# ruiminshen/yolo2-pytorch

Hardware: NVIDIA H100
Metric: 416x416 images/sec (higher is better)
Workload: dtype f16

## Files before the change

yolo2-pytorch_b200/b200/engine.py:

```python
import os

import torch

from . import ops

STRICT_KEEP = {'layers1.0': 'aw', 'layers1.2': 'aw', 'layers1.4': 'a', 'passthrough': 'aw', 'layers3.0': 'aw'}
PRECISIONS = ('fast', 'strict')


class OperandCache(dict):

    def fetch(self, key, tensors, build, extra=()):
        ver = tuple((t.data_ptr(), t._version) for t in tensors) + tuple(extra)
        hit = self.get(key)
        if hit is None or hit[0] != ver:
            hit = self[key] = (ver, build())
        return hit[1]


def epilogue_tensors(bn, bias=None):
    ts = () if bias is None else (bias,)
    return ts if bn is None else ts + (bn.weight, bn.bias, bn.running_mean, bn.running_var)


# ... 126 lines not shown

class DarknetEngine(object):
    def __init__(self, dnn):
        def unit(m):
            return ConvUnit(m.conv, m.bn if m.has_bn else None, m.has_act)

        self.units1, self.pools1, self._k1 = [], [], []
        mods = list(dnn.layers1)
        for i, m in enumerate(mods):
            if m.is_pool:
                continue
            self.units1.append(unit(m))
            self.pools1.append(i + 1 < len(mods) and mods[i + 1].is_pool)
            self._k1.append('layers1.%d' % i)
        self.units2 = [unit(m) for m in dnn.layers2 if not m.is_pool]
        self._k2 = ['layers2.%d' % i for i, m in enumerate(dnn.layers2) if not m.is_pool]
        self.unit_pt = unit(dnn.passthrough)
        self.units3 = [unit(m) for m in dnn.layers3]
        self.plans = {}
        if not self.pools1[0]:
            raise RuntimeError('Darknet: layers1.0 must be followed by MaxPool2d (fused first-layer kernel)')
        self.precision = 'fast'
        self.set_precision(os.environ.get('YB_PRECISION', 'fast'))

    def unit_keys(self):
        return self._k1 + self._k2 + ['passthrough', 'layers3.0', 'layers3.1']

    def set_precision(self, precision, keep=None):
        if precision not in PRECISIONS:
            raise ValueError('precision must be one of %s' % (PRECISIONS,))
        keep = STRICT_KEEP if keep is None else keep
        units = dict(zip(self.unit_keys(), self.all_units()))
        for key, u in units.items():
            k = keep.get(key, '') if precision == 'strict' else 'aw'
            u.split_a, u.split_w, u.out_lo = 'a' not in k, 'w' not in k, False
        units[self._k1[0]].split_a = units[self._k1[0]].split_w = False
        units[self._k1[1]].split_a = False
        chain1 = self.units1
        for prev, nxt in zip(chain1[:-1], chain1[1:]):
            prev.out_lo = nxt.split_a
        chain1[-1].out_lo = self.unit_pt.split_a or self.units2[0].split_a
        for prev, nxt in zip(self.units2[:-1], self.units2[1:]):
            prev.out_lo = nxt.split_a
        self.units2[-1].out_lo = self.unit_pt.out_lo = self.units3[0].split_a
        self.units3[0].out_lo = self.units3[1].split_a
        chain1[0].out_lo = False
# ... 30 lines not shown
        if u8:
            b, h, w, c = x.shape
        else:
            b, c, h, w = x.shape
        if c != 3 or h % 32 or w % 32:
            raise ValueError('Darknet expects fp32 [B,3,H,W] or uint8 [B,H,W,3] with H, W multiples of 32, got %s' % (tuple(x.shape),))
        x = x.contiguous() if u8 else x.contiguous().float()
        self.refresh()
        p = self.plan(b, h, w, x.device, plan_id)
        if self.precision == 'strict':
            return self._forward_strict(x, u8, p, conv_flags, collect)

        def conv(u, src, dst, **kw):
            return ops.conv_bn_act(src, u.w16, u.scale, u.shift, u.slope, out=dst, flags=conv_flags, ref=ref, workspace=p.workspace, **kw)

        u0 = self.units1[0]
        conv0 = ops.conv0_u8_bn_leaky_pool if u8 else ops.conv0_bn_leaky_pool
        cur = conv0(x, u0.w16, u0.scale, u0.shift, u0.slope, out=p.a0)
        if collect is not None:
            collect['layers1.0(pooled)'] = cur
        x1 = None
        last1 = self.units1[-1]
        for u, (out, pooled), key in zip(self.units1[1:], p.l1, self._k1[1:]):
            fuse_pool = (pooled is not None and u is not last1 and collect is None and not ref and u.cin == 32 and u.ksize == 3
                         and u.cout <= 64 and (conv_flags & (ops.CONV_NO_SMALLK | ops.CONV_C32_IM2COL)) == 0 and conv_flags < 256)
            if fuse_pool:
                ops.conv_bn_act(cur, u.w16, u.scale, u.shift, u.slope, out=pooled, flags=conv_flags | ops.CONV_POOL2X2)
                cur = pooled
                continue
            conv(u, cur, out)
            if collect is not None:
                collect[key] = out
            x1 = out
            cur = ops.maxpool2x2(out, out=pooled) if pooled is not None else out
        conv(self.unit_pt, x1, p.pt)
        if collect is not None:
            collect['passthrough'] = p.pt
        ops.reorg_f16(p.pt, p.cat, 0)
        cur = ops.maxpool2x2(x1, out=p.x1_pool)
        for u, out, key in zip(self.units2[:-1], p.l2, self._k2):
            conv(u, cur, out)
            if collect is not None:
                collect[key] = out
            cur = out
        conv(self.units2[-1], cur, p.cat, y_ch_off=self.unit_pt.cout * 4)
        conv(self.units3[0], p.cat, p.l3)
        conv(self.units3[1], p.l3, p.feature, out_mode=ops.OUT_F32_NCHW)
        if collect is not None:
            collect['cat'] = p.cat
            collect['layers3.0'] = p.l3
# ... 63 lines not shown
```

yolo2-pytorch_b200/b200/ops.py:

```python
import ctypes

import torch

from . import lib as _l

OUT_F16_NHWC, OUT_F32_NCHW = 0, 1
CONV_A_TILED, CONV_WIDE_N = 1, 2
CONV_NO_STREAMK, CONV_FORCE_STREAMK, CONV_NO_SMALLK, CONV_PLAIN_STORE = 8, 1 << 30, 1 << 28, 1 << 29
CONV_POOL2X2, CONV_C32_IM2COL, CONV_C32_SWAP = 16, 32, 64
FILTER_THRESHOLD, FILTER_FIX, FILTER_NONE = 0, 1, 2


launch_count = 0


def _ck(rc, what):
    global launch_count
    _l.check(rc, what)
    launch_count += 1


def conv_force_bn(bn):
    return bn << 8

# ... 108 lines not shown
        fn_name = 'yb_conv_bn_act_fwd_ws'
    fn = getattr(_l.load(), fn_name)
    args = [_p(x), _p(w), _p(scale), _p(shift), float(slope), _p(out), batch, height, width, cin, cout, k, x_ld, y_ld, y_ch_off, out_mode]
    if fn_name != 'yb_conv_ref_fwd':
        args.append(flags)
    if fn_name == 'yb_conv_bn_act_fwd_ws':
        _req(workspace, torch.uint8, 'workspace')
        args += [_p(workspace), workspace.numel()]
    args.append(_s())
    _ck(fn(*args), fn_name)


def conv_workspace(device='cuda'):
    return torch.zeros(int(_l.load().yb_conv_workspace_bytes()), dtype=torch.uint8, device=device)


CONV_KERNELS = ('conv_igemm_kernel', 'conv_wide_kernel', 'conv_c32_kernel')


def conv_choice(batch, height, width, cin, cout, k, out_mode=OUT_F16_NHWC, flags=0, workspace=True):
    out = (ctypes.c_int * 6)()
    _l.check(_l.load().yb_conv_choice(batch, height, width, cin, cout, k, out_mode, flags, int(bool(workspace)), ctypes.byref(out)),
             'yb_conv_choice')
    return dict(kernel=CONV_KERNELS[out[0]], bk=out[1], bn=out[2], rows=out[3], streamk=bool(out[4]), grid=out[5])


def conv_bn_act(x, w, scale, shift, slope, out=None, out_mode=OUT_F16_NHWC, y_ch_off=0, cin=None, flags=0, ref=False, workspace=None):
    _req(x, torch.float16, 'x'); _req(w, torch.float16, 'w'); _req(scale, torch.float32, 'scale'); _req(shift, torch.float32, 'shift')
    b, h, wd, x_ld = x.shape
    cout, k, _, wcin = w.shape
    cin = wcin if cin is None else cin
    if cin != wcin:
        raise ValueError('weight Cin %d != %d' % (wcin, cin))
    if out is None:
        oh, ow = (h // 2, wd // 2) if (flags & CONV_POOL2X2) else (h, wd)
        out = (torch.empty(b, oh, ow, cout, dtype=torch.float16, device=x.device) if out_mode == OUT_F16_NHWC
               else torch.empty(b, cout, h, wd, dtype=torch.float32, device=x.device))
    if out_mode == OUT_F16_NHWC:
        _req(out, torch.float16, 'out')
        y_ld = out.shape[-1]
    else:
        _req(out, torch.float32, 'out')
        y_ld = 0
    _conv_common('yb_conv_ref_fwd' if ref else 'yb_conv_bn_act_fwd', x, w, scale, shift, slope, out, b, h, wd, cin, cout, k, x_ld, y_ld,
                 y_ch_off, out_mode, flags, workspace=None if ref else workspace)
    return out


def conv2d_out_size(size, k, stride, pad):
    return (size + 2 * pad - k) // stride + 1


def conv2d_choice(batch, height, width, cin, cout, kh, kw, stride=1, pad=(0, 0), out_mode=OUT_F16_NHWC, flags=0, workspace=True):
    out = (ctypes.c_int * 6)()
    _l.check(_l.load().yb_conv2d_choice(batch, height, width, cin, cout, kh, kw, stride, pad[0], pad[1], out_mode, flags, int(bool(workspace)),
                                        ctypes.byref(out)), 'yb_conv2d_choice')
    return dict(kernel=CONV_KERNELS[out[0]], bk=out[1], bn=out[2], rows=out[3], streamk=bool(out[4]), grid=out[5])


def conv2d_bn_act(x, w, scale, shift, slope, stride=1, pad=(0, 0), out=None, out_mode=OUT_F16_NHWC, y_ch_off=0, cin=None, flags=0, workspace=None):
    _req(x, torch.float16, 'x'); _req(w, torch.float16, 'w'); _req(scale, torch.float32, 'scale'); _req(shift, torch.float32, 'shift')
    b, h, wd, x_ld = x.shape
    cout, kh, kw, wcin = w.shape
    cin = wcin if cin is None else cin
    if cin != wcin:
        raise ValueError('weight Cin %d != %d' % (wcin, cin))
    oh, ow = conv2d_out_size(h, kh, stride, pad[0]), conv2d_out_size(wd, kw, stride, pad[1])
    if out is None:
        out = (torch.empty(b, oh, ow, cout, dtype=torch.float16, device=x.device) if out_mode == OUT_F16_NHWC
               else torch.empty(b, cout, oh, ow, dtype=torch.float32, device=x.device))
    if out_mode == OUT_F16_NHWC:
        _req(out, torch.float16, 'out')
        y_ld = out.shape[-1]
    else:
        _req(out, torch.float32, 'out')
        y_ld = 0
    ws_ptr, ws_bytes = (None, 0) if workspace is None else (_p(_req(workspace, torch.uint8, 'workspace')), workspace.numel())
    _ck(_l.load().yb_conv2d_bn_act_fwd(_p(x), _p(w), _p(scale), _p(shift), float(slope), _p(out), b, h, wd, cin, cout, kh, kw, stride, pad[0], pad[1],
                                       x_ld, y_ld, y_ch_off, out_mode, flags, ws_ptr, ws_bytes, _s()), 'yb_conv2d_bn_act_fwd')
    return out
# ... 380 lines not shown
```

yolo2-pytorch_b200/csrc/conv_igemm.cu:

```cuda
#include "yb_common.h"
#include "yb_ptx.cuh"
#include <stdlib.h>

namespace yb {

struct ConvParams {
  int m_total;
  int height, width;
  int cin, cout;
  int kh, kw, pad_h, pad_w, stride;
  int in_h, in_w;
  int kb_per_tap;
  int num_kb;
  int m_tiles, n_tiles;
  int a_im2col;
  const float* scale;
  const float* shift;
  float slope;
  void* y;
  long long y_ld;
  int y_ch_off;
  int out_mode;
  int hw;
  int skip;
// ... 545 lines not shown
      acc_phase ^= 1;
    }
    if (p.tma_store && lane == 0) tma_store_wait<0>();
  }
}

template <int BN, int BK, int MT>
__global__ void __launch_bounds__(kThreads, 1)
conv_igemm_kernel(const __grid_constant__ CUtensorMap tmap_a, const __grid_constant__ CUtensorMap tmap_b,
                  const __grid_constant__ CUtensorMap tmap_y, const ConvParams p) {
  conv_igemm_body<BN, BK, MT, false>(tmap_a, tmap_b, tmap_y, p, PreAct{nullptr, nullptr, 0});
}

template <int BN, int BK, int MT>
__global__ void __launch_bounds__(kThreads, 1)
conv_preact_kernel(const __grid_constant__ CUtensorMap tmap_a, const __grid_constant__ CUtensorMap tmap_b,
                   const __grid_constant__ CUtensorMap tmap_y, const ConvParams p, const PreAct pre) {
  conv_igemm_body<BN, BK, MT, true>(tmap_a, tmap_b, tmap_y, p, pre);
}

constexpr int kWideThreads = 384;
constexpr int kWideRows = 256;
constexpr int kWideBN = 128;

template <int BK>
struct WideCfg {
  static constexpr int kSwizzle = BK * 2;
  static constexpr int kABytes = kWideRows * BK * 2;
  static constexpr int kBBytes = kWideBN * BK * 2;
  static constexpr int kStageBytes = kABytes + kBBytes;
  static constexpr int kOutBytes = 128 * 128;
  static constexpr int kTableBytes = kWideBN * 2 * 4;
  static constexpr int kFixedBytes = 2 * kOutBytes + kTableBytes + 1024  + 256 ;
  static constexpr int kStages = ((kSmemLimit - kFixedBytes) / kStageBytes) > 8 ? 8 : ((kSmemLimit - kFixedBytes) / kStageBytes);
  static constexpr int kSmemBytes = kStages * kStageBytes + kFixedBytes;
  static constexpr int kWsFloats = kWideRows * kWideBN;
  static_assert(kStages >= (BK == 64 ? 4 : 8), "shared memory budget: the epilogue's slices and table must not cost a pipeline stage");
};

template <int BK>
__global__ void __launch_bounds__(kWideThreads, 1)
conv_wide_kernel(const __grid_constant__ CUtensorMap tmap_a, const __grid_constant__ CUtensorMap tmap_b,
                 const __grid_constant__ CUtensorMap tmap_y, const ConvParams p) {
  using Cfg = WideCfg<BK>;
  constexpr int kStages = Cfg::kStages;
  extern __shared__ uint8_t smem_raw[];
  const uint32_t smem_base = (smem_u32(smem_raw) + 1023u) & ~1023u;
  const uint32_t smem_a = smem_base;
  const uint32_t smem_b = smem_base + kStages * Cfg::kABytes;
  const uint32_t smem_o = smem_base + kStages * Cfg::kStageBytes;
  const uint32_t table = smem_o + 2 * Cfg::kOutBytes;
  const uint32_t bar_full = table + Cfg::kTableBytes;
  const uint32_t bar_empty = bar_full + 8 * kStages;
  const uint32_t bar_slice_full = bar_empty + 8 * kStages;
  const uint32_t bar_slice_empty = bar_slice_full + 16;
  const int num_tiles = p.m_tiles * p.n_tiles;
  const int unit_id = static_cast<int>(blockIdx.x);
  const int num_units = static_cast<int>(gridDim.x);

  if (threadIdx.x == 0) {
    for (int i = 0; i < kStages; ++i) {
      mbar_init(bar_full + 8 * i, 1);
      mbar_init(bar_empty + 8 * i, 8);
    }
    for (int c = 0; c < 2; ++c) {
      mbar_init(bar_slice_full + 8 * c, 4);
      mbar_init(bar_slice_empty + 8 * c, 1);
    }
    fence_mbar_init();
    fence_proxy_async_smem();
    tma_prefetch_desc(&tmap_a);
    tma_prefetch_desc(&tmap_b);
    tma_prefetch_desc(&tmap_y);
  }
  __syncthreads();
  pdl_trigger();
  pdl_wait();

  if (threadIdx.x < 128) {
    setmaxnreg_dec<40>();
    if (threadIdx.x == 0) {
      int stage = 0;
      uint32_t phase = 0;
      int tr_p = 0;
      for (WorkIter it(p, unit_id, num_units, num_tiles); it.valid(); it.next()) {
        const int n_tile = it.tile % p.n_tiles;
        const int m_cta = (it.tile / p.n_tiles) * kWideRows;
        const int img = m_cta / p.hw;
        const int rem = m_cta - img * p.hw;
        const int oh = rem / p.width;
        const int h0 = oh * p.stride - p.pad_h;
        const int w0 = (rem - oh * p.width) * p.stride - p.pad_w;
        for (int kb = it.kb0; kb < it.kb1; ++kb) {
          const int tap = kb / p.kb_per_tap;
          const int c0 = (kb - tap * p.kb_per_tap) * BK;
          const int ca = c0 >= p.a_wrap ? c0 - p.a_wrap : c0;
          const int r = tap / p.kw;
          const int s = tap - r * p.kw;
          mbar_wait(bar_empty + 8 * stage, phase ^ 1, p.dbg, 0x600 | stage);
          YB_TRACE(0, tr_p); ++tr_p;
          const uint32_t full = bar_full + 8 * stage;
          mbar_arrive_expect_tx(full, Cfg::kStageBytes);
          const uint32_t dst = smem_a + stage * Cfg::kABytes;
          if (p.a_im2col) tma_load_im2col_4d(dst, &tmap_a, full, ca, w0, h0, img, static_cast<uint16_t>(s), static_cast<uint16_t>(r));
          else tma_load_2d(dst, &tmap_a, full, ca, m_cta);
          tma_load_2d(smem_b + stage * Cfg::kBBytes, &tmap_b, full, tap * p.cin + c0, n_tile * kWideBN);
          if (++stage == kStages) { stage = 0; phase ^= 1; }
        }
      }
    } else if (threadIdx.x == 32 || threadIdx.x == 64) {
      const int c = (threadIdx.x >> 5) - 1;
      const uint32_t slice = smem_o + c * Cfg::kOutBytes;
      uint32_t sph = 0;
      for (WorkIter it(p, unit_id, num_units, num_tiles); it.valid(); it.next()) {
        if (it.kb1 < p.num_kb) continue;
        const int n0 = (it.tile % p.n_tiles) * kWideBN;
        const int m_base = (it.tile / p.n_tiles) * kWideRows + c * 128;
        for (int h = 0; h < 2; ++h) {
          mbar_wait(bar_slice_full + 8 * c, sph, p.dbg, 0x900 | c);
#pragma unroll
          for (int c2 = 0; c2 < 2; ++c2) {
            if (n0 + c2 * 64 < p.cout) {
#pragma unroll
              for (int g = 0; g < 2; ++g) {
                const int row = m_base + h * 64 + g * 32;
                if (row < p.m_total) tma_store_2d(&tmap_y, slice + c2 * 8192 + g * 4096, n0 + c2 * 64, row);
              }
            }
          }
          tma_store_commit();
          tma_store_wait_read<0>();
          mbar_arrive(bar_slice_empty + 8 * c);
          sph ^= 1;
        }
      }
      tma_store_wait<0>();
    }
    return;
  }
  setmaxnreg_inc<232>();
  const int cw = (threadIdx.x >> 7) - 1;
// ... 69 lines not shown
      if (leader) {
        for (int j = sk_lo; j < static_cast<int>(blockIdx.x); ++j) {
          uint32_t spins = 0;
          uint64_t t0 = 0;
          while (ld_acquire_gpu(p.flags + j) == 0u) {
            if ((++spins & 0x3FFu) == 0) {
              const uint64_t now = globaltimer_ns();
              if (t0 == 0) t0 = now;
              if (now - t0 > 4000000000ull) {
                if (p.dbg != nullptr) { p.dbg[0] = 0x0BAD0800; p.dbg[1] = static_cast<int>(blockIdx.x); p.dbg[2] = j; p.dbg[3] = tile; __threadfence_system(); }
                __trap();
              }
            }
          }
        }
      }
      asm volatile("bar.sync 1, 256;" ::: "memory");
    }
    if (!sk_dump) {
      asm volatile("bar.sync 1, 256;" ::: "memory");
      asm volatile("st.shared.f32 [%0], %1;" :: "r"(table + 4 * te), "f"(tab) : "memory");
      asm volatile("bar.sync 1, 256;" ::: "memory");
    }
#pragma unroll
    for (int h = 0; h < 2; ++h) {
      if (h == 1) {
        wgmma_wait<0>();
        fence_regs(acc[1]);
        if (leader) YB_TRACE(2, tr_t);
        release_prev();
      }
      if (sk_dump) {
        float4* dst = reinterpret_cast<float4*>(p.ws + static_cast<size_t>(blockIdx.x) * Cfg::kWsFloats) + (cw * 32 + 16 * h) * 128 + t;
#pragma unroll
        for (int g = 0; g < 16; ++g) dst[g * 128] = make_float4(acc[h][4 * g], acc[h][4 * g + 1], acc[h][4 * g + 2], acc[h][4 * g + 3]);
        continue;
      }
      for (int j = sk_lo; j < (sk_collect ? static_cast<int>(blockIdx.x) : 0); ++j) {
        const float4* src = reinterpret_cast<const float4*>(p.ws + static_cast<size_t>(j) * Cfg::kWsFloats) + (cw * 32 + 16 * h) * 128 + t;
#pragma unroll
        for (int g = 0; g < 16; ++g) {
          const float4 a = __ldcg(src + g * 128);
          acc[h][4 * g] += a.x; acc[h][4 * g + 1] += a.y; acc[h][4 * g + 2] += a.z; acc[h][4 * g + 3] += a.w;
        }
      }
      uint32_t pk[32];
#pragma unroll
      for (int c2 = 0; c2 < 2; ++c2) {
#pragma unroll
        for (int jj = 0; jj < 8; ++jj) {
          const float4 ss = tab4[c2 * 32 + 4 * jj + (lane & 3)];
#pragma unroll
          for (int hh = 0; hh < 2; ++hh) {
            const int j = c2 * 8 + jj;
            float x0 = acc[h][4 * j + 2 * hh] * ss.x + ss.z;
            float x1 = acc[h][4 * j + 2 * hh + 1] * ss.y + ss.w;
            x0 = x0 > 0.f ? x0 : x0 * p.slope;
            x1 = x1 > 0.f ? x1 : x1 * p.slope;
            __half2 v = __floats2half2_rn(x0, x1);
            pk[16 * c2 + 2 * jj + hh] = *reinterpret_cast<uint32_t*>(&v);
          }
        }
      }
      mbar_wait(bar_slice_empty + 8 * cw, sph ^ 1, p.dbg, 0xA00 | cw);
#pragma unroll
      for (int c2 = 0; c2 < 2; ++c2)
#pragma unroll
        for (int jj = 0; jj < 8; ++jj)
#pragma unroll
          for (int hh = 0; hh < 2; ++hh) {
            const int r = warp * 16 + (lane >> 2) + hh * 8;
            const uint32_t addr = slice + c2 * 8192 + r * 128 + ((jj ^ (r & 7)) << 4) + 4 * (lane & 3);
            asm volatile("st.shared.b32 [%0], %1;" :: "r"(addr), "r"(pk[16 * c2 + 2 * jj + hh]) : "memory");
          }
      fence_proxy_async_smem();
      __syncwarp();
      if (lane == 0) mbar_arrive(bar_slice_full + 8 * cw);
      sph ^= 1;
    }
    if (sk_dump) {
      __threadfence();
      asm volatile("bar.sync 1, 256;" ::: "memory");
      if (leader) st_release_gpu(p.flags + blockIdx.x, 1u);
      continue;
    }
    if (leader) YB_TRACE(2, tr_t + 1);
    if (sk_collect) {
      asm volatile("bar.sync 1, 256;" ::: "memory");
      for (int j = sk_lo + t + 128 * cw; j < static_cast<int>(blockIdx.x); j += 256) p.flags[j] = 0u;
    }
  }
}

struct C32Params {
  int batch, height, width, cout;
  int tiles_w, tiles_h, num_tiles;
  const float* scale;
  const float* shift;
  float slope;
  int pool;
  int swap_lbo;
  int skip;
  int* dbg;
  unsigned long long* trace;
  double* stats;
};

struct C32Cfg {
  static constexpr int TH = 16, TW = 8, HH = TH + 2, HW = TW + 2;
  static constexpr int kPlaneData = HH * HW * 16;
  static constexpr int kPlane = (kPlaneData + 127) / 128 * 128;
  static constexpr int kHalo = 4 * kPlane;
  static constexpr int kStages = 4;
  static constexpr int BN = 64;
// ... 210 lines not shown
      }
      if (et == 0) { YB_TRACE(2, tr); ++tr; }
    }
    if (gt == 0) tma_store_wait<0>();
    if (p.stats != nullptr) {
      asm volatile("bar.sync 8, %0;" :: "n"(Cfg::kEpiThreads) : "memory");
      for (int i = et; i < p.cout; i += Cfg::kEpiThreads) {
        atomicAdd(p.stats + i, static_cast<double>(ep_stats[i]));
        atomicAdd(p.stats + p.cout + i, static_cast<double>(ep_stats[BN + i]));
      }
    }
  }
}

constexpr long long kSkFlagBytes = 4096;
constexpr long long kSkSlotBytes = kWideRows * kWideBN * 4;
long long conv_workspace_bytes() { return kSkFlagBytes + kSkSlotBytes * sm_count(); }

constexpr int kKernelIgemm = 0;
constexpr int kKernelWide = 1;
constexpr int kKernelC32 = 2;
struct ConvChoice {
  int kernel, bk, bn, mt, streamk, grid;
};

static unsigned long long* g_conv_trace = nullptr;
void conv_set_trace(void* dev_ptr) { g_conv_trace = static_cast<unsigned long long*>(dev_ptr); }

typedef CUresult (*EncodeTiledFn)(CUtensorMap*, CUtensorMapDataType, cuuint32_t, void*, const cuuint64_t*, const cuuint64_t*,
                                  const cuuint32_t*, const cuuint32_t*, CUtensorMapInterleave, CUtensorMapSwizzle,
                                  CUtensorMapL2promotion, CUtensorMapFloatOOBfill);
typedef CUresult (*EncodeIm2colFn)(CUtensorMap*, CUtensorMapDataType, cuuint32_t, void*, const cuuint64_t*, const cuuint64_t*,
                                   const int*, const int*, cuuint32_t, cuuint32_t, const cuuint32_t*, CUtensorMapInterleave,
                                   CUtensorMapSwizzle, CUtensorMapL2promotion, CUtensorMapFloatOOBfill);

static int get_encoders(EncodeTiledFn* tiled, EncodeIm2colFn* im2col) {
  static EncodeTiledFn s_tiled = nullptr;
  static EncodeIm2colFn s_im2col = nullptr;
  if (s_tiled == nullptr || s_im2col == nullptr) {
    void* f0 = nullptr;
    void* f1 = nullptr;
    cudaDriverEntryPointQueryResult q0, q1;
    YB_CUDA(cudaGetDriverEntryPoint("cuTensorMapEncodeTiled", &f0, cudaEnableDefault, &q0));
    YB_CUDA(cudaGetDriverEntryPoint("cuTensorMapEncodeIm2col", &f1, cudaEnableDefault, &q1));
    if (f0 == nullptr || f1 == nullptr || q0 != cudaDriverEntryPointSuccess || q1 != cudaDriverEntryPointSuccess)
      return fail(YB_ERR_DRIVER, "cuTensorMapEncode* driver entry points unavailable");
// ... 51 lines not shown
  using Cfg = WideCfg<BK>;
  static bool attr_set = false;
  if (!attr_set) {
    YB_CUDA(cudaFuncSetAttribute(conv_wide_kernel<BK>, cudaFuncAttributeMaxDynamicSharedMemorySize, Cfg::kSmemBytes));
    attr_set = true;
  }
  cudaLaunchConfig_t cfg;
  memset(&cfg, 0, sizeof(cfg));
  cudaLaunchAttribute attr[1];
  int nattr = 0;
  static const int use_pdl = getenv("YB_PDL") ? atoi(getenv("YB_PDL")) : 0;
  if (use_pdl) {
    attr[nattr].id = cudaLaunchAttributeProgrammaticStreamSerialization;
    attr[nattr].val.programmaticStreamSerializationAllowed = 1;
    ++nattr;
  }
  cfg.gridDim = dim3(grid);
  cfg.blockDim = dim3(kWideThreads);
  cfg.dynamicSmemBytes = Cfg::kSmemBytes;
  cfg.stream = stream;
  cfg.attrs = attr; cfg.numAttrs = nattr;
  YB_CUDA(cudaLaunchKernelEx(&cfg, conv_wide_kernel<BK>, ta, tb, ty, p));
  return check_launch("conv_wide_kernel");
}

template <int BK>
static int dispatch_conv(int bn, int mt, int grid, const CUtensorMap& ta, const CUtensorMap& tb, const CUtensorMap& ty, const ConvParams& p,
                         const PreAct* pre, cudaStream_t stream) {
  if (mt == 2 && bn == 128) return launch_wide<BK>(ta, tb, ty, p, grid, stream);
  if (mt == 2) return launch_conv<64, BK, 2>(ta, tb, ty, p, pre, stream);
  if (bn == 64) return launch_conv<64, BK, 1>(ta, tb, ty, p, pre, stream);
  return launch_conv<128, BK, 1>(ta, tb, ty, p, pre, stream);
}

static int conv_c32_forward(const void* x, const void* w, const float* scale, const float* shift, float slope, void* y, int batch,
                            int height, int width, int cout, int x_ld, long long y_ld, int y_ch_off, int pool, int flags, double* stats,
                            cudaStream_t stream) {
  using Cfg = C32Cfg;
  EncodeTiledFn enc_tiled;
  EncodeIm2colFn enc_im2col;
  int rc = get_encoders(&enc_tiled, &enc_im2col);
  if (rc) return rc;
  YB_REQUIRE(!pool || (height % 2 == 0 && width % 2 == 0), "conv: fused 2x2 max-pool needs even H and W");
  C32Params p;
  p.batch = batch; p.height = height; p.width = width; p.cout = cout;
  p.tiles_w = (width + Cfg::TW - 1) / Cfg::TW;
// ... 48 lines not shown
  }
  const int grid = p.num_tiles < sm_count() ? p.num_tiles : sm_count();
  conv_c32_kernel<<<grid, Cfg::kThreads, Cfg::kSmemBytes, stream>>>(tx, tw, ty, p);
  return check_launch("conv_c32_kernel");
}

constexpr double kKbNsIm2col = 240.0;
constexpr double kKbNsTiled = 100.0;
constexpr double kFeedBytesPerNs = 130.0;
constexpr double kEpiNsPerOut = 0.15;
constexpr double kWideEpiNsPerOut = 0.04;
constexpr double kSkNs = 16000.0;
constexpr double kSkNsWide = 9000.0;
int conv_choose(int batch, int height, int width, int cin, int cout, int kh, int kw, int stride, int pad_h, int pad_w, int a_channels, int out_mode,
                int flags, bool workspace_ok, bool stats, bool lo, bool pre, ConvChoice* out) {
  ConvChoice c;
  memset(&c, 0, sizeof(c));
  const int sms = sm_count();
  const bool split = a_channels != cin || lo;
  const bool same3x3 = kh == 3 && kw == 3 && stride == 1 && pad_h == 1 && pad_w == 1;
  const bool im2col_cost = !(kh == 1 && kw == 1 && stride == 1);
  if (!split && cin == 32 && same3x3 && cout <= 64 && out_mode == 0 && ((flags >> 28) & 1) == 0 && ((flags >> 5) & 1) == 0 && ((flags >> 8) & 0xFFFF) == 0) {
    const long long tiles = static_cast<long long>(batch) * ((width + C32Cfg::TW - 1) / C32Cfg::TW) * ((height + C32Cfg::TH - 1) / C32Cfg::TH);
    c.kernel = kKernelC32; c.bk = 32; c.bn = C32Cfg::BN; c.mt = 1;
    c.grid = static_cast<int>(tiles < sms ? tiles : sms);
    *out = c;
    return 0;
  }
  if ((flags >> 4) & 1) return fail(YB_ERR_UNSUPPORTED, "conv: YB_CONV_POOL2X2 is only implemented for the Cin = 32 3x3 layer");
  const int bk = (cin % 64 == 0 && a_channels % 64 == 0) ? 64 : 32;
  const bool sk_possible = !stats && workspace_ok && (flags & 8) == 0;
  const bool sk_force = sk_possible && ((flags >> 30) & 1);
  const bool wide_ok = out_mode == 0 && !lo && !stats && !pre && ((flags >> 24) & 0xF) == 0 && ((flags >> 29) & 1) == 0;
  const int force_bn = (flags >> 8) & 0x3FF;
  const int force_mt = (flags >> 20) & 0x3;
  const int force_pair = (flags >> 22) & 0x3;
  YB_REQUIRE(force_pair != 2, "conv: CTA-pair tiles need two-CTA tensor-core instructions, which sm_90 does not have");
  YB_REQUIRE(!force_bn || ((force_bn == 64 || force_bn == 128) && (force_mt != 2 || force_bn == 64 || wide_ok)),
             "conv: BLOCK_N=%d x %d M-subtiles is not a tile shape of this launch (64 x 1, 128 x 1, 64 x 2; 128 x 2 for fp16 NHWC "
             "outputs without residual or statistics)", force_bn, force_mt ? force_mt : 1);
  const long long m_total = static_cast<long long>(batch) * height * width;
  const int num_kb = kh * kw * (cin / bk);
  double best = 1e300;
  for (int cbn = 64; cbn <= 128; cbn *= 2) {
    if (force_bn && cbn != force_bn) continue;
    if (!force_bn && cbn > 64 && cbn / 2 >= cout) continue;
    for (int cmt = 1; cmt <= 2; ++cmt) {
      if (force_mt && cmt != force_mt) continue;
      const bool cwide = cmt * cbn > 128;
      if (cwide && !wide_ok) continue;
      const int rows_tile = BM * cmt;
      const double tiles = static_cast<double>((m_total + rows_tile - 1) / rows_tile) * ((cout + cbn - 1) / cbn);
      const double rounds = static_cast<double>((static_cast<long long>(tiles) + sms - 1) / sms);
      const double kb_ns = (im2col_cost ? kKbNsIm2col : kKbNsTiled) + (cmt * BM + cbn) * bk * 2.0 / kFeedBytesPerNs;
      const double main_ns = num_kb * kb_ns;
      const double outs = static_cast<double>(rows_tile) * cbn;
      const double tile_ns = cwide ? main_ns + outs * kWideEpiNsPerOut : (main_ns > outs * kEpiNsPerOut ? main_ns : outs * kEpiNsPerOut);
      double t = rounds * tile_ns;
      int csk = 0;
      if (sk_possible) {
        const double units = tiles * num_kb;
        const double per_cta = static_cast<double>((static_cast<long long>(units) + sms - 1) / sms);
        const double tsk = per_cta * kb_ns + (cwide ? kSkNsWide : kSkNs);
        const bool ok = per_cta >= 4.0 && num_kb >= 2;
        const bool idle = tiles <= sms / 2;
        if (ok && (sk_force || (idle && tsk < 0.93 * t))) { t = tsk; csk = 1; }
      }
      if (sk_force && !csk) continue;
      if (t < best * 0.9999 || (t <= best * 1.0001 && cbn > c.bn)) { best = t; c.bn = cbn; c.mt = cmt; c.streamk = csk; }
    }
  }
  if (c.bn == 0) { c.bn = force_bn ? force_bn : 128; c.mt = force_mt ? force_mt : 1; c.streamk = 0; }
  YB_REQUIRE((c.bn == 64 || c.bn == 128) && (c.mt == 1 || c.mt == 2) && (c.mt * c.bn <= 128 || wide_ok), "conv: tile %d x %d", c.bn, c.mt);
  c.kernel = c.mt * c.bn > 128 ? kKernelWide : kKernelIgemm;
  c.bk = bk;
  const long long tiles = ((m_total + BM * c.mt - 1) / (BM * c.mt)) * ((cout + c.bn - 1) / c.bn);
  c.grid = c.streamk ? sms : static_cast<int>(tiles < sms ? tiles : sms);
  *out = c;
  return 0;
}

static int conv_geometry(int in_h, int in_w, int kh, int kw, int stride, int pad_h, int pad_w, int* out_h, int* out_w) {
  YB_REQUIRE(kh >= 1 && kh <= 7 && kw >= 1 && kw <= 7, "conv2d: kernel %d x %d (1..7 on each axis)", kh, kw);
  YB_REQUIRE(stride == 1 || stride == 2, "conv2d: stride %d (1 or 2)", stride);
  YB_REQUIRE(pad_h >= 0 && pad_h < kh && pad_w >= 0 && pad_w < kw, "conv2d: padding (%d, %d) for a %d x %d kernel (0 <= pad < k)", pad_h, pad_w, kh,
             kw);
  YB_REQUIRE(in_h > 0 && in_w > 0 && in_h + 2 * pad_h >= kh && in_w + 2 * pad_w >= kw, "conv2d: %d x %d input gives an empty output", in_h, in_w);
  *out_h = (in_h + 2 * pad_h - kh) / stride + 1;
  *out_w = (in_w + 2 * pad_w - kw) / stride + 1;
  return 0;
}

int conv2d_choice(int batch, int in_h, int in_w, int cin, int cout, int kh, int kw, int stride, int pad_h, int pad_w, int out_mode, int flags,
                  int with_workspace, int* out) {
  YB_REQUIRE(out != nullptr && batch > 0 && cin > 0 && cin % 32 == 0 && cout > 0, "conv_choice: bad shape");
  int oh = 0, ow = 0;
  int rc = conv_geometry(in_h, in_w, kh, kw, stride, pad_h, pad_w, &oh, &ow);
  if (rc) return rc;
// ... 42 lines not shown
  if (out_mode == 0) {
    YB_REQUIRE(cout % 8 == 0 && y_ld % 8 == 0 && y_ch_off % 8 == 0 && (reinterpret_cast<uintptr_t>(y) & 15) == 0,
               "conv: fp16 NHWC output needs Cout, y_ld, y_ch_off multiples of 8 and a 16B aligned pointer");
  }
  const long long m_total_ll = static_cast<long long>(batch) * height * width;
  YB_REQUIRE(m_total_ll < (1ll << 31) - kWideRows && static_cast<long long>(batch) * in_h * in_w < (1ll << 31), "conv: too many pixels");
  const bool ws_ok = workspace != nullptr && workspace_bytes >= conv_workspace_bytes() && (reinterpret_cast<uintptr_t>(workspace) & 255) == 0;
  ConvChoice ch;
  rc = conv_choose(batch, height, width, cin, cout, kh, kw, stride, pad_h, pad_w, a_channels, out_mode, flags, ws_ok, stats != nullptr, lo_ch_off >= 0,
                   pre, &ch);
  if (rc) return rc;
  YB_REQUIRE(!pre || ch.kernel == kKernelIgemm, "conv_preact: no pre-activation form of kernel %d", ch.kernel);
  if (ch.kernel == kKernelC32)
    return conv_c32_forward(x, w, scale, shift, slope, y, batch, height, width, cout, x_ld, y_ld, y_ch_off, (flags >> 4) & 1, flags, stats, stream);
  const int bk = ch.bk, bn = ch.bn, mt = ch.mt, streamk = ch.streamk;
  static const int k1x1_im2col = getenv("YB_CONV_1X1_IM2COL") ? atoi(getenv("YB_CONV_1X1_IM2COL")) : 0;
  const int a_im2col = !plain_1x1 ? 1 : ((k1x1_im2col && !(flags & 1) && !pre) ? 1 : 0);

  EncodeTiledFn enc_tiled;
  EncodeIm2colFn enc_im2col;
  rc = get_encoders(&enc_tiled, &enc_im2col);
  if (rc) return rc;

  ConvParams p;
  p.m_total = static_cast<int>(m_total_ll);
  p.height = height; p.width = width; p.cin = cin; p.cout = cout;
  p.kh = kh; p.kw = kw; p.pad_h = pad_h; p.pad_w = pad_w; p.stride = stride; p.in_h = in_h; p.in_w = in_w;
  p.kb_per_tap = cin / bk;
  p.num_kb = kh * kw * p.kb_per_tap;
  const int rows_tile = BM * mt;
  p.m_tiles = (p.m_total + rows_tile - 1) / rows_tile;
  p.n_tiles = (cout + bn - 1) / bn;
  p.a_im2col = a_im2col;
  p.scale = scale; p.shift = shift; p.slope = slope;
  p.y = y; p.y_ld = y_ld; p.y_ch_off = y_ch_off; p.out_mode = out_mode;
  p.hw = height * width;
  p.dbg = debug_word_device();
  p.trace = g_conv_trace;
  p.skip = (flags >> 24) & 0xF;
  p.streamk = streamk;
  p.stats = stats;
  p.tma_store = 0;
  p.a_wrap = a_channels;
  p.lo_off = lo_ch_off >= 0 ? static_cast<long long>(lo_ch_off - y_ch_off) : 0;
  p.sk_base = 0; p.sk_rem = 0; p.ws = nullptr; p.flags = nullptr;
  if (streamk) {
    const long long units = static_cast<long long>(p.m_tiles) * p.n_tiles * p.num_kb;
    YB_REQUIRE(units < (1ll << 31), "conv: stream-K unit count overflows");
    p.sk_base = static_cast<int>(units / sm_count());
    p.sk_rem = static_cast<int>(units % sm_count());
    p.flags = static_cast<unsigned*>(workspace);
    p.ws = reinterpret_cast<float*>(static_cast<char*>(workspace) + kSkFlagBytes);
  }

  const CUtensorMapSwizzle swz = (bk == 64) ? CU_TENSOR_MAP_SWIZZLE_128B : CU_TENSOR_MAP_SWIZZLE_64B;
  alignas(64) CUtensorMap ta, tb;
  CUresult cr;
  const int a_rows = BM * mt;
  if (a_im2col) {
    const cuuint64_t dims[4] = {static_cast<cuuint64_t>(a_channels), static_cast<cuuint64_t>(in_w), static_cast<cuuint64_t>(in_h),
                                static_cast<cuuint64_t>(batch)};
    const cuuint64_t strides[3] = {static_cast<cuuint64_t>(x_ld) * 2, static_cast<cuuint64_t>(x_ld) * 2 * in_w,
                                   static_cast<cuuint64_t>(x_ld) * 2 * in_w * in_h};
    const int lower[2] = {-pad_w, -pad_h};
    const int upper[2] = {pad_w - (kw - 1), pad_h - (kh - 1)};
    const cuuint32_t estr[4] = {1, static_cast<cuuint32_t>(stride), static_cast<cuuint32_t>(stride), 1};
    cr = enc_im2col(&ta, CU_TENSOR_MAP_DATA_TYPE_FLOAT16, 4, const_cast<void*>(x), dims, strides, lower, upper,
                    static_cast<cuuint32_t>(bk), static_cast<cuuint32_t>(a_rows), estr, CU_TENSOR_MAP_INTERLEAVE_NONE, swz, CU_TENSOR_MAP_L2_PROMOTION_L2_128B,
                    CU_TENSOR_MAP_FLOAT_OOB_FILL_NONE);
    if (cr != CUDA_SUCCESS) return fail(YB_ERR_DRIVER, "cuTensorMapEncodeIm2col failed (%d)", static_cast<int>(cr));
    int drv = 0;
    cudaDriverGetVersion(&drv);
    const unsigned long long span_bytes = static_cast<unsigned long long>(x_ld) * 2ull * in_w * in_h * batch;
    if (drv <= 13010 && span_bytes < 131072ull) reinterpret_cast<uint64_t*>(&ta)[1] &= ~(1ull << 21);
  } else {
    const cuuint64_t dims[2] = {static_cast<cuuint64_t>(a_channels), static_cast<cuuint64_t>(p.m_total)};
    const cuuint64_t strides[1] = {static_cast<cuuint64_t>(x_ld) * 2};
    const cuuint32_t box[2] = {static_cast<cuuint32_t>(bk), static_cast<cuuint32_t>(a_rows)};
    const cuuint32_t estr[2] = {1, 1};
    cr = enc_tiled(&ta, CU_TENSOR_MAP_DATA_TYPE_FLOAT16, 2, const_cast<void*>(x), dims, strides, box, estr,
                   CU_TENSOR_MAP_INTERLEAVE_NONE, swz, CU_TENSOR_MAP_L2_PROMOTION_L2_128B, CU_TENSOR_MAP_FLOAT_OOB_FILL_NONE);
    if (cr != CUDA_SUCCESS) return fail(YB_ERR_DRIVER, "cuTensorMapEncodeTiled(A) failed (%d)", static_cast<int>(cr));
  }
  {
    const cuuint64_t k_total = static_cast<cuuint64_t>(kh) * kw * cin;
    const cuuint64_t dims[2] = {k_total, static_cast<cuuint64_t>(cout)};
    const cuuint64_t strides[1] = {k_total * 2};
    const cuuint32_t box[2] = {static_cast<cuuint32_t>(bk), static_cast<cuuint32_t>(bn)};
    const cuuint32_t estr[2] = {1, 1};
    cr = enc_tiled(&tb, CU_TENSOR_MAP_DATA_TYPE_FLOAT16, 2, const_cast<void*>(w), dims, strides, box, estr,
                   CU_TENSOR_MAP_INTERLEAVE_NONE, swz, CU_TENSOR_MAP_L2_PROMOTION_L2_256B, CU_TENSOR_MAP_FLOAT_OOB_FILL_NONE);
    if (cr != CUDA_SUCCESS) return fail(YB_ERR_DRIVER, "cuTensorMapEncodeTiled(W) failed (%d)", static_cast<int>(cr));
  }

  alignas(64) CUtensorMap ty;
  memset(&ty, 0, sizeof(ty));
  p.tma_store = (out_mode == 0 && lo_ch_off < 0 && ((flags >> 29) & 1) == 0) ? 1 : 0;
  if (p.tma_store) {
    const cuuint64_t dims[2] = {static_cast<cuuint64_t>(cout), static_cast<cuuint64_t>(p.m_total)};
    const cuuint64_t strides[1] = {static_cast<cuuint64_t>(y_ld) * 2};
    const cuuint32_t box[2] = {64, 32};
    const cuuint32_t estr[2] = {1, 1};
    cr = enc_tiled(&ty, CU_TENSOR_MAP_DATA_TYPE_FLOAT16, 2, static_cast<__half*>(y) + y_ch_off, dims, strides, box, estr,
                   CU_TENSOR_MAP_INTERLEAVE_NONE, CU_TENSOR_MAP_SWIZZLE_128B, CU_TENSOR_MAP_L2_PROMOTION_NONE, CU_TENSOR_MAP_FLOAT_OOB_FILL_NONE);
    if (cr != CUDA_SUCCESS) return fail(YB_ERR_DRIVER, "cuTensorMapEncodeTiled(Y) failed (%d)", static_cast<int>(cr));
  }
  if (bk == 64) return dispatch_conv<64>(bn, mt, ch.grid, ta, tb, ty, p, pre ? &pre_act : nullptr, stream);
  return dispatch_conv<32>(bn, mt, ch.grid, ta, tb, ty, p, pre ? &pre_act : nullptr, stream);
}

int conv_igemm_forward(const void* x, const void* w, const float* scale, const float* shift, float slope, void* y, int batch,
                       int height, int width, int cin, int cout, int ksize, int x_ld, long long y_ld, int y_ch_off, int out_mode,
                       int flags, void* workspace, long long workspace_bytes, double* stats, int a_channels, int lo_ch_off,
                       const float* pre_scale, const float* pre_shift, int pre_relu, cudaStream_t stream) {
  YB_REQUIRE(ksize == 1 || ksize == 3, "conv: ksize %d unsupported (1 or 3)", ksize);
  return conv2d_forward(x, w, scale, shift, slope, y, batch, height, width, cin, cout, ksize, ksize, 1, (ksize - 1) / 2, (ksize - 1) / 2, x_ld, y_ld,
                        y_ch_off, out_mode, flags, workspace, workspace_bytes, stats, a_channels, lo_ch_off, pre_scale, pre_shift, pre_relu, stream);
}

__global__ void conv_ref_kernel(const __half* __restrict__ x, const __half* __restrict__ w, ConvParams p, int x_ld) {
  const long long idx = static_cast<long long>(blockIdx.x) * blockDim.x + threadIdx.x;
  const long long total = static_cast<long long>(p.m_total) * p.cout;
  if (idx >= total) return;
  const int co = static_cast<int>(idx % p.cout);
  const int row = static_cast<int>(idx / p.cout);
  const int img = row / p.hw;
  const int pix = row - img * p.hw;
  const int h = pix / p.width;
  const int wq = pix - h * p.width;
// ... 40 lines not shown
```

Measured before the change: 18660.

## Fuse 2x2 max-pool into the wide 256x128 implicit-GEMM conv kernel

Adds a pooled variant of the wide conv kernel. It loads four im2col tensor maps, one per pool offset, each covering a quarter of the rows, then reduces the four conv outputs with half2 max in the epilogue before storing the pooled NHWC result. It is used in the layers1 chain whenever the dispatcher picks the wide kernel, which removes the full-resolution conv output write and the separate maxpool launch and read. In exchange the pooled form turns off stream-K and uses only one output slice consumer, which may lower utilisation on layers where the tile count is small.

Result: faster. 19400 (median of 6 runs) (+3.9%).

```diff
diff --git a/yolo2-pytorch_b200/b200/engine.py b/yolo2-pytorch_b200/b200/engine.py
--- a/yolo2-pytorch_b200/b200/engine.py
+++ b/yolo2-pytorch_b200/b200/engine.py
@@ -172,6 +172,20 @@
             raise RuntimeError('Darknet: layers1.0 must be followed by MaxPool2d (fused first-layer kernel)')
         self.precision = 'fast'
         self.set_precision(os.environ.get('YB_PRECISION', 'fast'))
+        self.fuse_wide_pool = True
+        self._pool_ok = {}
+
+    def _pooled_form(self, u, x, conv_flags):
+        b, h, w, _ = x.shape
+        key = (u.cin, u.cout, u.ksize, b, h, w, conv_flags)
+        ok = self._pool_ok.get(key)
+        if ok is None:
+            try:
+                ok = ops.conv_choice(b, h, w, u.cin, u.cout, u.ksize, flags=conv_flags | ops.CONV_POOL2X2)['kernel'] == 'conv_wide_kernel'
+            except RuntimeError:
+                ok = False
+            self._pool_ok[key] = ok
+        return ok
 
     def unit_keys(self):
         return self._k1 + self._k2 + ['passthrough', 'layers3.0', 'layers3.1']
@@ -248,10 +262,11 @@
         x1 = None
         last1 = self.units1[-1]
         for u, (out, pooled), key in zip(self.units1[1:], p.l1, self._k1[1:]):
-            fuse_pool = (pooled is not None and u is not last1 and collect is None and not ref and u.cin == 32 and u.ksize == 3
-                         and u.cout <= 64 and (conv_flags & (ops.CONV_NO_SMALLK | ops.CONV_C32_IM2COL)) == 0 and conv_flags < 256)
+            fuse_pool = pooled is not None and u is not last1 and collect is None and not ref and (
+                (u.cin == 32 and u.ksize == 3 and u.cout <= 64 and (conv_flags & (ops.CONV_NO_SMALLK | ops.CONV_C32_IM2COL)) == 0
+                 and conv_flags < 256) or (self.fuse_wide_pool and self._pooled_form(u, cur, conv_flags)))
             if fuse_pool:
-                ops.conv_bn_act(cur, u.w16, u.scale, u.shift, u.slope, out=pooled, flags=conv_flags | ops.CONV_POOL2X2)
+                ops.conv_bn_act(cur, u.w16, u.scale, u.shift, u.slope, out=pooled, flags=conv_flags | ops.CONV_POOL2X2, workspace=p.workspace)
                 cur = pooled
                 continue
             conv(u, cur, out)
diff --git a/yolo2-pytorch_b200/b200/ops.py b/yolo2-pytorch_b200/b200/ops.py
--- a/yolo2-pytorch_b200/b200/ops.py
+++ b/yolo2-pytorch_b200/b200/ops.py
@@ -154,7 +154,8 @@
     out = (ctypes.c_int * 6)()
     _l.check(_l.load().yb_conv_choice(batch, height, width, cin, cout, k, out_mode, flags, int(bool(workspace)), ctypes.byref(out)),
              'yb_conv_choice')
-    return dict(kernel=CONV_KERNELS[out[0]], bk=out[1], bn=out[2], rows=out[3], streamk=bool(out[4]), grid=out[5])
+    return dict(kernel=CONV_KERNELS[out[0]], bk=out[1], bn=out[2], rows=out[3], streamk=bool(out[4]), grid=out[5],
+                pooled=bool(flags & CONV_POOL2X2))
 
 
 def conv_bn_act(x, w, scale, shift, slope, out=None, out_mode=OUT_F16_NHWC, y_ch_off=0, cin=None, flags=0, ref=False, workspace=None):
@@ -174,6 +175,12 @@
     else:
         _req(out, torch.float32, 'out')
         y_ld = 0
+    if flags & CONV_POOL2X2:
+        if ref:
+            raise ValueError('conv_bn_act: the CUDA-core reference has no fused max-pool')
+        if out.dim() != 4 or tuple(out.shape[:3]) != (b, h // 2, wd // 2) or y_ch_off < 0 or y_ch_off + cout > y_ld:
+            raise ValueError('conv_bn_act: pooled out must be [%d,%d,%d,y_ld] with y_ch_off + Cout <= y_ld, got %s at y_ch_off %d'
+                             % (b, h // 2, wd // 2, tuple(out.shape), y_ch_off))
     _conv_common('yb_conv_ref_fwd' if ref else 'yb_conv_bn_act_fwd', x, w, scale, shift, slope, out, b, h, wd, cin, cout, k, x_ld, y_ld,
                  y_ch_off, out_mode, flags, workspace=None if ref else workspace)
     return out
@@ -187,7 +194,8 @@
     out = (ctypes.c_int * 6)()
     _l.check(_l.load().yb_conv2d_choice(batch, height, width, cin, cout, kh, kw, stride, pad[0], pad[1], out_mode, flags, int(bool(workspace)),
                                         ctypes.byref(out)), 'yb_conv2d_choice')
-    return dict(kernel=CONV_KERNELS[out[0]], bk=out[1], bn=out[2], rows=out[3], streamk=bool(out[4]), grid=out[5])
+    return dict(kernel=CONV_KERNELS[out[0]], bk=out[1], bn=out[2], rows=out[3], streamk=bool(out[4]), grid=out[5],
+                pooled=bool(flags & CONV_POOL2X2))
 
 
 def conv2d_bn_act(x, w, scale, shift, slope, stride=1, pad=(0, 0), out=None, out_mode=OUT_F16_NHWC, y_ch_off=0, cin=None, flags=0, workspace=None):
diff --git a/yolo2-pytorch_b200/csrc/conv_igemm.cu b/yolo2-pytorch_b200/csrc/conv_igemm.cu
--- a/yolo2-pytorch_b200/csrc/conv_igemm.cu
+++ b/yolo2-pytorch_b200/csrc/conv_igemm.cu
@@ -591,6 +591,12 @@
 constexpr int kWideThreads = 384;
 constexpr int kWideRows = 256;
 constexpr int kWideBN = 128;
+constexpr int kWidePoolRows = kWideRows / 4;
+
+__device__ __forceinline__ uint32_t hmax2_u32(uint32_t a, uint32_t b) {
+  const __half2 m = __hmax2(*reinterpret_cast<const __half2*>(&a), *reinterpret_cast<const __half2*>(&b));
+  return *reinterpret_cast<const uint32_t*>(&m);
+}
 
 template <int BK>
 struct WideCfg {
@@ -607,10 +613,9 @@
   static_assert(kStages >= (BK == 64 ? 4 : 8), "shared memory budget: the epilogue's slices and table must not cost a pipeline stage");
 };
 
-template <int BK>
-__global__ void __launch_bounds__(kWideThreads, 1)
-conv_wide_kernel(const __grid_constant__ CUtensorMap tmap_a, const __grid_constant__ CUtensorMap tmap_b,
-                 const __grid_constant__ CUtensorMap tmap_y, const ConvParams p) {
+template <int BK, bool kPool>
+__device__ __forceinline__ void conv_wide_body(const CUtensorMap* const (&tmap_a)[4], const CUtensorMap& tmap_b, const CUtensorMap& tmap_y,
+                                               const ConvParams p) {
   using Cfg = WideCfg<BK>;
   constexpr int kStages = Cfg::kStages;
   extern __shared__ uint8_t smem_raw[];
@@ -634,11 +639,15 @@
     }
     for (int c = 0; c < 2; ++c) {
       mbar_init(bar_slice_full + 8 * c, 4);
-      mbar_init(bar_slice_empty + 8 * c, 1);
+      if constexpr (kPool) mbar_init(bar_slice_empty + 8 * c, c == 1 ? 4 : 1);
+      else mbar_init(bar_slice_empty + 8 * c, 1);
     }
     fence_mbar_init();
     fence_proxy_async_smem();
-    tma_prefetch_desc(&tmap_a);
+    tma_prefetch_desc(tmap_a[0]);
+    if constexpr (kPool) {
+      for (int b = 1; b < 4; ++b) tma_prefetch_desc(tmap_a[b]);
+    }
     tma_prefetch_desc(&tmap_b);
     tma_prefetch_desc(&tmap_y);
   }
@@ -654,7 +663,7 @@
       int tr_p = 0;
       for (WorkIter it(p, unit_id, num_units, num_tiles); it.valid(); it.next()) {
         const int n_tile = it.tile % p.n_tiles;
-        const int m_cta = (it.tile / p.n_tiles) * kWideRows;
+        const int m_cta = (it.tile / p.n_tiles) * (kPool ? kWidePoolRows : kWideRows);
         const int img = m_cta / p.hw;
         const int rem = m_cta - img * p.hw;
         const int oh = rem / p.width;
@@ -671,21 +680,28 @@
           const uint32_t full = bar_full + 8 * stage;
           mbar_arrive_expect_tx(full, Cfg::kStageBytes);
           const uint32_t dst = smem_a + stage * Cfg::kABytes;
-          if (p.a_im2col) tma_load_im2col_4d(dst, &tmap_a, full, ca, w0, h0, img, static_cast<uint16_t>(s), static_cast<uint16_t>(r));
-          else tma_load_2d(dst, &tmap_a, full, ca, m_cta);
+          if constexpr (kPool) {
+#pragma unroll
+            for (int b = 0; b < 4; ++b)
+              tma_load_im2col_4d(dst + b * kWidePoolRows * BK * 2, tmap_a[b], full, ca, w0 + (b & 1), h0 + (b >> 1), img, static_cast<uint16_t>(s),
+                                 static_cast<uint16_t>(r));
+          } else {
+            if (p.a_im2col) tma_load_im2col_4d(dst, tmap_a[0], full, ca, w0, h0, img, static_cast<uint16_t>(s), static_cast<uint16_t>(r));
+            else tma_load_2d(dst, tmap_a[0], full, ca, m_cta);
+          }
           tma_load_2d(smem_b + stage * Cfg::kBBytes, &tmap_b, full, tap * p.cin + c0, n_tile * kWideBN);
           if (++stage == kStages) { stage = 0; phase ^= 1; }
         }
       }
-    } else if (threadIdx.x == 32 || threadIdx.x == 64) {
+    } else if (threadIdx.x == 32 || (!kPool && threadIdx.x == 64)) {
       const int c = (threadIdx.x >> 5) - 1;
       const uint32_t slice = smem_o + c * Cfg::kOutBytes;
       uint32_t sph = 0;
       for (WorkIter it(p, unit_id, num_units, num_tiles); it.valid(); it.next()) {
         if (it.kb1 < p.num_kb) continue;
         const int n0 = (it.tile % p.n_tiles) * kWideBN;
-        const int m_base = (it.tile / p.n_tiles) * kWideRows + c * 128;
-        for (int h = 0; h < 2; ++h) {
+        const int m_base = kPool ? (it.tile / p.n_tiles) * kWidePoolRows : (it.tile / p.n_tiles) * kWideRows + c * 128;
+        for (int h = 0; h < (kPool ? 1 : 2); ++h) {
           mbar_wait(bar_slice_full + 8 * c, sph, p.dbg, 0x900 | c);
 #pragma unroll
           for (int c2 = 0; c2 < 2; ++c2) {
@@ -801,6 +817,7 @@
       asm volatile("st.shared.f32 [%0], %1;" :: "r"(table + 4 * te), "f"(tab) : "memory");
       asm volatile("bar.sync 1, 256;" ::: "memory");
     }
+    uint32_t pk_dx0[kPool ? 32 : 1];
 #pragma unroll
     for (int h = 0; h < 2; ++h) {
       if (h == 1) {
@@ -841,6 +858,32 @@
           }
         }
       }
+      if constexpr (kPool) {
+        if (h == 0) {
+#pragma unroll
+          for (int i = 0; i < 32; ++i) pk_dx0[i] = pk[i];
+          continue;
+        }
+#pragma unroll
+        for (int i = 0; i < 32; ++i) pk[i] = hmax2_u32(pk_dx0[i], pk[i]);
+        if (cw == 0) {
+          mbar_wait(bar_slice_full + 8, sph, p.dbg, 0xB00);
+#pragma unroll
+          for (int c2 = 0; c2 < 2; ++c2)
+#pragma unroll
+            for (int jj = 0; jj < 8; ++jj)
+#pragma unroll
+              for (int hh = 0; hh < 2; ++hh) {
+                const int r = warp * 16 + (lane >> 2) + hh * 8;
+                const uint32_t addr = smem_o + Cfg::kOutBytes + c2 * 8192 + r * 128 + ((jj ^ (r & 7)) << 4) + 4 * (lane & 3);
+                uint32_t v;
+                asm volatile("ld.shared.b32 %0, [%1];" : "=r"(v) : "r"(addr) : "memory");
+                pk[16 * c2 + 2 * jj + hh] = hmax2_u32(pk[16 * c2 + 2 * jj + hh], v);
+              }
+          __syncwarp();
+          if (lane == 0) mbar_arrive(bar_slice_empty + 8);
+        }
+      }
       mbar_wait(bar_slice_empty + 8 * cw, sph ^ 1, p.dbg, 0xA00 | cw);
 #pragma unroll
       for (int c2 = 0; c2 < 2; ++c2)
@@ -869,6 +912,23 @@
       for (int j = sk_lo + t + 128 * cw; j < static_cast<int>(blockIdx.x); j += 256) p.flags[j] = 0u;
     }
   }
+}
+
+template <int BK>
+__global__ void __launch_bounds__(kWideThreads, 1)
+conv_wide_kernel(const __grid_constant__ CUtensorMap tmap_a, const __grid_constant__ CUtensorMap tmap_b,
+                 const __grid_constant__ CUtensorMap tmap_y, const ConvParams p) {
+  const CUtensorMap* const ta[4] = {&tmap_a, &tmap_a, &tmap_a, &tmap_a};
+  conv_wide_body<BK, false>(ta, tmap_b, tmap_y, p);
+}
+
+template <int BK>
+__global__ void __launch_bounds__(kWideThreads, 1)
+conv_wide_pool_kernel(const __grid_constant__ CUtensorMap tmap_a0, const __grid_constant__ CUtensorMap tmap_a1,
+                      const __grid_constant__ CUtensorMap tmap_a2, const __grid_constant__ CUtensorMap tmap_a3,
+                      const __grid_constant__ CUtensorMap tmap_b, const __grid_constant__ CUtensorMap tmap_y, const ConvParams p) {
+  const CUtensorMap* const ta[4] = {&tmap_a0, &tmap_a1, &tmap_a2, &tmap_a3};
+  conv_wide_body<BK, true>(ta, tmap_b, tmap_y, p);
 }
 
 struct C32Params {
@@ -1125,6 +1185,7 @@
 constexpr int kKernelC32 = 2;
 struct ConvChoice {
   int kernel, bk, bn, mt, streamk, grid;
+  int pool;
 };
 
 static unsigned long long* g_conv_trace = nullptr;
@@ -1222,6 +1283,19 @@
   cfg.attrs = attr; cfg.numAttrs = nattr;
   YB_CUDA(cudaLaunchKernelEx(&cfg, conv_wide_kernel<BK>, ta, tb, ty, p));
   return check_launch("conv_wide_kernel");
+}
+
+template <int BK>
+static int launch_wide_pool(const CUtensorMap (&ta)[4], const CUtensorMap& tb, const CUtensorMap& ty, const ConvParams& p, int grid,
+                            cudaStream_t stream) {
+  using Cfg = WideCfg<BK>;
+  static bool attr_set = false;
+  if (!attr_set) {
+    YB_CUDA(cudaFuncSetAttribute(conv_wide_pool_kernel<BK>, cudaFuncAttributeMaxDynamicSharedMemorySize, Cfg::kSmemBytes));
+    attr_set = true;
+  }
+  conv_wide_pool_kernel<BK><<<grid, kWideThreads, Cfg::kSmemBytes, stream>>>(ta[0], ta[1], ta[2], ta[3], tb, ty, p);
+  return check_launch("conv_wide_pool_kernel");
 }
 
 template <int BK>
@@ -1316,14 +1390,20 @@
   const bool im2col_cost = !(kh == 1 && kw == 1 && stride == 1);
   if (!split && cin == 32 && same3x3 && cout <= 64 && out_mode == 0 && ((flags >> 28) & 1) == 0 && ((flags >> 5) & 1) == 0 && ((flags >> 8) & 0xFFFF) == 0) {
     const long long tiles = static_cast<long long>(batch) * ((width + C32Cfg::TW - 1) / C32Cfg::TW) * ((height + C32Cfg::TH - 1) / C32Cfg::TH);
-    c.kernel = kKernelC32; c.bk = 32; c.bn = C32Cfg::BN; c.mt = 1;
+    c.kernel = kKernelC32; c.bk = 32; c.bn = C32Cfg::BN; c.mt = 1; c.pool = (flags >> 4) & 1;
     c.grid = static_cast<int>(tiles < sms ? tiles : sms);
     *out = c;
     return 0;
   }
-  if ((flags >> 4) & 1) return fail(YB_ERR_UNSUPPORTED, "conv: YB_CONV_POOL2X2 is only implemented for the Cin = 32 3x3 layer");
+  const bool pool = (flags >> 4) & 1;
+  if (pool) {
+    if (!(same3x3 && height % 2 == 0 && width % 2 == 0 && out_mode == 0 && !split && !stats && !pre))
+      return fail(YB_ERR_UNSUPPORTED, "conv: YB_CONV_POOL2X2 needs a 3x3 same-padded stride-1 layer with even H and W, fp16 NHWC output and "
+                                      "plain operands");
+    if ((flags >> 30) & 1) return fail(YB_ERR_UNSUPPORTED, "conv: the fused 2x2 max-pool has no stream-K form");
+  }
   const int bk = (cin % 64 == 0 && a_channels % 64 == 0) ? 64 : 32;
-  const bool sk_possible = !stats && workspace_ok && (flags & 8) == 0;
+  const bool sk_possible = !stats && !pool && workspace_ok && (flags & 8) == 0;
   const bool sk_force = sk_possible && ((flags >> 30) & 1);
   const bool wide_ok = out_mode == 0 && !lo && !stats && !pre && ((flags >> 24) & 0xF) == 0 && ((flags >> 29) & 1) == 0;
   const int force_bn = (flags >> 8) & 0x3FF;
@@ -1368,6 +1448,10 @@
   YB_REQUIRE((c.bn == 64 || c.bn == 128) && (c.mt == 1 || c.mt == 2) && (c.mt * c.bn <= 128 || wide_ok), "conv: tile %d x %d", c.bn, c.mt);
   c.kernel = c.mt * c.bn > 128 ? kKernelWide : kKernelIgemm;
   c.bk = bk;
+  if (pool && c.kernel != kKernelWide)
+    return fail(YB_ERR_UNSUPPORTED, "conv: the fused 2x2 max-pool runs on the 256 x 128 two-consumer tile only; this launch takes %d x %d tiles",
+                BM * c.mt, c.bn);
+  c.pool = pool;
   const long long tiles = ((m_total + BM * c.mt - 1) / (BM * c.mt)) * ((cout + c.bn - 1) / c.bn);
   c.grid = c.streamk ? sms : static_cast<int>(tiles < sms ? tiles : sms);
   *out = c;
@@ -1456,13 +1540,15 @@
   rc = get_encoders(&enc_tiled, &enc_im2col);
   if (rc) return rc;
 
+  const bool pooled = ch.pool != 0;
+  if (pooled) { height /= 2; width /= 2; }
   ConvParams p;
-  p.m_total = static_cast<int>(m_total_ll);
+  p.m_total = static_cast<int>(static_cast<long long>(batch) * height * width);
   p.height = height; p.width = width; p.cin = cin; p.cout = cout;
-  p.kh = kh; p.kw = kw; p.pad_h = pad_h; p.pad_w = pad_w; p.stride = stride; p.in_h = in_h; p.in_w = in_w;
+  p.kh = kh; p.kw = kw; p.pad_h = pad_h; p.pad_w = pad_w; p.stride = pooled ? 2 : stride; p.in_h = in_h; p.in_w = in_w;
   p.kb_per_tap = cin / bk;
   p.num_kb = kh * kw * p.kb_per_tap;
-  const int rows_tile = BM * mt;
+  const int rows_tile = pooled ? kWidePoolRows : BM * mt;
   p.m_tiles = (p.m_total + rows_tile - 1) / rows_tile;
   p.n_tiles = (cout + bn - 1) / bn;
   p.a_im2col = a_im2col;
@@ -1488,25 +1574,30 @@
   }
 
   const CUtensorMapSwizzle swz = (bk == 64) ? CU_TENSOR_MAP_SWIZZLE_128B : CU_TENSOR_MAP_SWIZZLE_64B;
-  alignas(64) CUtensorMap ta, tb;
+  alignas(64) CUtensorMap ta_pos[4];
+  alignas(64) CUtensorMap tb;
+  CUtensorMap& ta = ta_pos[0];
   CUresult cr;
-  const int a_rows = BM * mt;
+  const int a_rows = pooled ? kWidePoolRows : BM * mt;
   if (a_im2col) {
     const cuuint64_t dims[4] = {static_cast<cuuint64_t>(a_channels), static_cast<cuuint64_t>(in_w), static_cast<cuuint64_t>(in_h),
                                 static_cast<cuuint64_t>(batch)};
     const cuuint64_t strides[3] = {static_cast<cuuint64_t>(x_ld) * 2, static_cast<cuuint64_t>(x_ld) * 2 * in_w,
                                    static_cast<cuuint64_t>(x_ld) * 2 * in_w * in_h};
-    const int lower[2] = {-pad_w, -pad_h};
-    const int upper[2] = {pad_w - (kw - 1), pad_h - (kh - 1)};
-    const cuuint32_t estr[4] = {1, static_cast<cuuint32_t>(stride), static_cast<cuuint32_t>(stride), 1};
-    cr = enc_im2col(&ta, CU_TENSOR_MAP_DATA_TYPE_FLOAT16, 4, const_cast<void*>(x), dims, strides, lower, upper,
-                    static_cast<cuuint32_t>(bk), static_cast<cuuint32_t>(a_rows), estr, CU_TENSOR_MAP_INTERLEAVE_NONE, swz, CU_TENSOR_MAP_L2_PROMOTION_L2_128B,
-                    CU_TENSOR_MAP_FLOAT_OOB_FILL_NONE);
-    if (cr != CUDA_SUCCESS) return fail(YB_ERR_DRIVER, "cuTensorMapEncodeIm2col failed (%d)", static_cast<int>(cr));
+    const cuuint32_t estr[4] = {1, static_cast<cuuint32_t>(p.stride), static_cast<cuuint32_t>(p.stride), 1};
     int drv = 0;
     cudaDriverGetVersion(&drv);
-    const unsigned long long span_bytes = static_cast<unsigned long long>(x_ld) * 2ull * in_w * in_h * batch;
-    if (drv <= 13010 && span_bytes < 131072ull) reinterpret_cast<uint64_t*>(&ta)[1] &= ~(1ull << 21);
+    for (int b = 0; b < (pooled ? 4 : 1); ++b) {
+      const int dx = pooled ? (b & 1) : 0, dy = pooled ? (b >> 1) : 0;
+      const int lower[2] = {dx - pad_w, dy - pad_h};
+      const int upper[2] = {dx + pad_w - (kw - 1) - (pooled ? 1 : 0), dy + pad_h - (kh - 1) - (pooled ? 1 : 0)};
+      cr = enc_im2col(&ta_pos[b], CU_TENSOR_MAP_DATA_TYPE_FLOAT16, 4, const_cast<void*>(x), dims, strides, lower, upper,
+                      static_cast<cuuint32_t>(bk), static_cast<cuuint32_t>(a_rows), estr, CU_TENSOR_MAP_INTERLEAVE_NONE, swz, CU_TENSOR_MAP_L2_PROMOTION_L2_128B,
+                      CU_TENSOR_MAP_FLOAT_OOB_FILL_NONE);
+      if (cr != CUDA_SUCCESS) return fail(YB_ERR_DRIVER, "cuTensorMapEncodeIm2col failed (%d)", static_cast<int>(cr));
+      const unsigned long long span_bytes = static_cast<unsigned long long>(x_ld) * 2ull * in_w * in_h * batch;
+      if (drv <= 13010 && span_bytes < 131072ull) reinterpret_cast<uint64_t*>(&ta_pos[b])[1] &= ~(1ull << 21);
+    }
   } else {
     const cuuint64_t dims[2] = {static_cast<cuuint64_t>(a_channels), static_cast<cuuint64_t>(p.m_total)};
     const cuuint64_t strides[1] = {static_cast<cuuint64_t>(x_ld) * 2};
@@ -1539,6 +1630,7 @@
                    CU_TENSOR_MAP_INTERLEAVE_NONE, CU_TENSOR_MAP_SWIZZLE_128B, CU_TENSOR_MAP_L2_PROMOTION_NONE, CU_TENSOR_MAP_FLOAT_OOB_FILL_NONE);
     if (cr != CUDA_SUCCESS) return fail(YB_ERR_DRIVER, "cuTensorMapEncodeTiled(Y) failed (%d)", static_cast<int>(cr));
   }
+  if (pooled) return bk == 64 ? launch_wide_pool<64>(ta_pos, tb, ty, p, ch.grid, stream) : launch_wide_pool<32>(ta_pos, tb, ty, p, ch.grid, stream);
   if (bk == 64) return dispatch_conv<64>(bn, mt, ch.grid, ta, tb, ty, p, pre ? &pre_act : nullptr, stream);
   return dispatch_conv<32>(bn, mt, ch.grid, ta, tb, ty, p, pre ? &pre_act : nullptr, stream);
 }
```
